# gildas-lormeau/zlib-streams-ts

Hardware: AMD Instinct MI355X
Metric: uncompressed MB/s, deflate-raw L6, 4096x64KiB batch at 1/2/4/8 GPUs (higher is better)
Workload: dtype u8; 1 GPU; 4096 x 65536 B text-corpus streams split across the GPUs, deflate-raw level 6; global_streams=4096, streams_per_gpu=4096, stream_bytes=65536, level=6, format=deflate-raw, compressed_bytes=91855591, parallelism=dp1

## Files before the change

zlib-streams-ts_amd/csrc/deflate_sweep.hip:

```cpp
#include <hip/hip_runtime.h>
#include "zs_common.h"
#include "zs_kernels.h"
#include "zs_sweep_ring.h"
#include "zs_sweep_long.h"
#include "zs_sweep_ends.h"
#include <type_traits>
#include <utility>

#define ZS_SW_WIN_WORDS ((ZS_SEG_WPOS + 258u + 20u + 3u) / 4u + 2u)
#define ZS_SW_RING 128u
#define ZS_SW_MW 320u
#ifndef ZS_SW_RUN_CAP
#define ZS_SW_RUN_CAP 16u
#endif

typedef __attribute__((address_space(3))) uint32_t zs_sw_lds_u32;
static __device__ __forceinline__ uint32_t sw_lds_addr(const void* p) {
  return (uint32_t)(uintptr_t)(const zs_sw_lds_u32*)p;
}

static __device__ __forceinline__ uint32_t sw_hash(uint32_t w) {
  return (((w & 0xffu) << 10) ^ (((w >> 8) & 0xffu) << 5) ^ ((w >> 16) & 0xffu)) & ZS_HASH_MASK;
}

#define ZS_BK_WPT (16384u / ZS_BK_THREADS)
#define ZS_BK_PPL (ZS_BK_THREADS / 64u)
#ifndef ZS_BK_PROF
#define ZS_BK_PROF 0
#endif
#if ZS_BK_PROF
__device__ unsigned long long zs_bk_stat[4];
extern "C" int zs_bucket_stats(unsigned long long* out) {
  return (int)hipMemcpyFromSymbol(out, HIP_SYMBOL(zs_bk_stat), sizeof(zs_bk_stat));
}
#define BK_MARK(i) do { if (threadIdx.x == 0) { const unsigned long long t_ = wall_clock64(); atomicAdd(&zs_bk_stat[i], t_ - bk_t); bk_t = t_; } } while (0)
#else
#define BK_MARK(i) do { } while (0)
#endif
#define ZS_BK_INFLIGHT 8
#define ZS_BK_CHUNK 2048u
#define ZS_BK_KEYS 256u
#define ZS_BK_HELPERS (ZS_BK_THREADS - 64u)
#define ZS_BK_EPT ((ZS_BK_CHUNK + ZS_BK_HELPERS - 1u) / ZS_BK_HELPERS)

static __device__ __forceinline__ void bk_lds_barrier() {
  asm volatile("s_waitcnt lgkmcnt(0)\n\ts_barrier" ::: "memory");
}

template <bool ORD>
__global__ __launch_bounds__(ZS_BK_THREADS) void zs_k_bucket(const uint8_t* __restrict__ in,
                                                            const uint64_t* __restrict__ in_off,
                                                            const uint32_t* __restrict__ in_len,
                                                            const uint64_t* __restrict__ pos_base,
                                                            const zs_sweep_seg* __restrict__ segs,
                                                            uint16_t* __restrict__ members, uint2* __restrict__ mres) {
  __shared__ uint32_t cnt[16384];
  __shared__ uint32_t part[ZS_BK_KEYS + ZS_BK_CHUNK / 2];
  static_assert(ZS_BK_KEYS + ZS_BK_CHUNK / 2 >= ZS_BK_THREADS, "part[] holds the scan's partial sums");
  __shared__ uint32_t stg[ZS_BK_CHUNK / 4 + 2];
  __shared__ uint16_t q[2][ZS_BK_CHUNK];
  const zs_sweep_seg G = segs[blockIdx.x];
  const int s = (int)G.s;
  const uint32_t nrel = in_len[s] - G.base;
  const uint32_t tid = threadIdx.x;
  const uint8_t* src = in + in_off[s] + G.base;
  uint16_t* mem = members + G.mb;
  uint2* out = mres + pos_base[s] + G.base;
  const uint32_t m = nrel > 2 ? min(nrel - 2, G.ohi) : 0u;
  const uint32_t n = min(nrel, m + 2u);
  if (nrel - m <= 2u)
    for (uint32_t p = m + tid; p < nrel; p += ZS_BK_THREADS) out[p] = make_uint2(0, 0);
  if (m == 0) return;
  for (uint32_t i = tid; i < 16384 / 4; i += ZS_BK_THREADS) reinterpret_cast<uint4*>(cnt)[i] = make_uint4(0, 0, 0, 0);
  const bool aligned = ((uintptr_t)src & 3u) == 0;
#if ZS_BK_PROF
  unsigned long long bk_t = wall_clock64();
  if (threadIdx.x == 0) atomicAdd(&zs_bk_stat[3], 1ull);
#endif
  __syncthreads();
  {
    uint32_t w[5], nw[5];
    auto load5 = [&](uint32_t p0, uint32_t* x) __attribute__((always_inline)) {
#pragma unroll
      for (int k = 0; k < 5; k++) x[k] = zs_load_word(src, n, p0 + 16 * tid + 4 * k);
    };
    load5(0, nw);
    for (uint32_t p0 = 0; p0 < m; p0 += 16 * ZS_BK_THREADS) {
#pragma unroll
      for (int k = 0; k < 5; k++) w[k] = nw[k];
      if (p0 + 16 * ZS_BK_THREADS < m) load5(p0 + 16 * ZS_BK_THREADS, nw);
#pragma unroll
      for (uint32_t j = 0; j < 16; j++) {
        const uint32_t p = p0 + 16 * tid + j;
        const uint32_t h = sw_hash(__builtin_amdgcn_alignbyte(w[(j >> 2) + 1], w[j >> 2], j & 3u));
        if (p < m) atomicAdd(&cnt[h >> 1], 1u << (16u * (h & 1u)));
      }
    }
  }
  __syncthreads();
  BK_MARK(0);
  {
    uint32_t sum = 0;
    for (uint32_t j = 0; j < ZS_BK_WPT; j++) {
      const uint32_t w = cnt[ZS_BK_WPT * tid + ((j + tid) & (ZS_BK_WPT - 1u))];
      sum += (w & 0xffffu) + (w >> 16);
    }
    part[tid] = sum;
    __syncthreads();
    if (tid < 64) {
      uint32_t v[ZS_BK_PPL], t = 0;
#pragma unroll
      for (uint32_t j = 0; j < ZS_BK_PPL; j++) { v[j] = part[ZS_BK_PPL * tid + j]; t += v[j]; }
      uint32_t x = t;
#pragma unroll
      for (int d = 1; d < 64; d <<= 1) {
        const uint32_t y = __shfl_up(x, d, 64);
        if (tid >= (uint32_t)d) x += y;
      }
      uint32_t run = x - t;
#pragma unroll
      for (uint32_t j = 0; j < ZS_BK_PPL; j++) { part[ZS_BK_PPL * tid + j] = run; run += v[j]; }
    }
    __syncthreads();
    uint32_t run = part[tid];
    for (uint32_t j = 0; j < ZS_BK_WPT; j++) {
      const uint32_t w = cnt[ZS_BK_WPT * tid + j];
      const uint32_t lo = w & 0xffffu;
      cnt[ZS_BK_WPT * tid + j] = run | ((run + lo) << 16);
      run += lo + (w >> 16);
    }
  }
  __syncthreads();
  BK_MARK(1);
  const uint32_t wave = tid >> 6, lane = tid & 63u;
  constexpr uint32_t PH = ZS_BK_CHUNK / (64 * ZS_BK_INFLIGHT);
  static_assert(PH == 4, "a chunk is four steps: count, scan, place, store");
  uint32_t* const kc = part;
  uint16_t* const srt = reinterpret_cast<uint16_t*>(part + ZS_BK_KEYS);
  if (tid < ZS_BK_KEYS) kc[tid] = 0;
  uint32_t sl[ZS_BK_EPT];
  const uint32_t ht = tid - 64u;
  constexpr uint32_t CW = ZS_BK_CHUNK / 4 / 64;
  uint32_t nxt[CW + 1];
  auto fetch = [&](uint32_t c0) {
#pragma unroll
    for (uint32_t i = 0; i <= CW; i++) {
      const uint32_t w = 64 * i + lane;
      const uint32_t at = c0 + 4 * w;
      uint32_t v = 0;
      if (w < ZS_BK_CHUNK / 4 + 2) {
        if (aligned && at + 4 <= n) v = *(const uint32_t*)(src + at);
        else
          for (uint32_t k = 0; k < 4; k++)
            if (at + k < n) v |= (uint32_t)src[at + k] << (8 * k);
      }
      nxt[i] = v;
    }
  };
  if (wave == 0) fetch(0);
  const uint32_t nch = (m + ZS_BK_CHUNK - 1) / ZS_BK_CHUNK;
  for (uint32_t c = 0; c <= nch; c++) {
    const uint32_t c0 = c * ZS_BK_CHUNK;
    const uint32_t c1 = min(m, c0 + ZS_BK_CHUNK);
    const uint32_t b0 = c0 - ZS_BK_CHUNK, cnt1 = min(m, c0) - b0;
    const uint16_t* const qp = q[(c - 1) & 1u];
#pragma unroll
    for (uint32_t ph = 0; ph < PH; ph++) {
    const uint32_t g0 = c0 + 64 * ZS_BK_INFLIGHT * ph;
    if (wave == 0 && c < nch) {
      if (ph == 0) {
        __builtin_amdgcn_s_waitcnt(0xc07f);
        __builtin_amdgcn_wave_barrier();
#pragma unroll
        for (uint32_t i = 0; i <= CW; i++)
          if (64 * i + lane < ZS_BK_CHUNK / 4 + 2) stg[64 * i + lane] = nxt[i];
        __builtin_amdgcn_s_waitcnt(0xc07f);
        __builtin_amdgcn_wave_barrier();
        if (c0 + ZS_BK_CHUNK < m) fetch(c0 + ZS_BK_CHUNK);
      }
      uint16_t* const qc = q[c & 1u];
      if (g0 < c1) {
        uint32_t a[ZS_BK_INFLIGHT], v[ZS_BK_INFLIGHT], sh[ZS_BK_INFLIGHT], e[ZS_BK_INFLIGHT], hh[ZS_BK_INFLIGHT];
#pragma unroll
        for (int j = 0; j < ZS_BK_INFLIGHT; j++) {
          const uint32_t p = g0 + 64 * j + lane;
          const uint32_t o = p - c0;
          const uint32_t h = sw_hash(__builtin_amdgcn_alignbyte(stg[(o >> 2) + 1], stg[o >> 2], o & 3u));
          hh[j] = h;
          sh[j] = 16u * (h & 1u);
          a[j] = sw_lds_addr(&cnt[h >> 1]);
          v[j] = p < c1 ? 1u << sh[j] : 0u;
        }
        if (!ORD) {
#pragma unroll
          for (int j = 0; j < ZS_BK_INFLIGHT; j++) {
            const uint32_t p = g0 + 64 * j + lane;
            const uint32_t h = hh[j];
            const uint64_t mm = zs_wave_match(h, p < c1);
            const uint32_t rank = (uint32_t)__builtin_popcountll(mm & ((1ull << lane) - 1ull));
            const uint32_t lead = mm ? (uint32_t)__builtin_ctzll(mm) : lane;
            uint32_t old = 0;
            if (p < c1 && lead == lane)
              old = atomicAdd(&cnt[h >> 1], (uint32_t)__builtin_popcountll(mm) << sh[j]);
            old = (uint32_t)__builtin_amdgcn_ds_bpermute((int)(lead * 4u), (int)old);
            e[j] = old + (rank << sh[j]);
          }
        } else {
        asm volatile(
            "ds_add_rtn_u32 %0, %8, %16\n\t"
            "ds_add_rtn_u32 %1, %9, %17\n\t"
            "ds_add_rtn_u32 %2, %10, %18\n\t"
            "ds_add_rtn_u32 %3, %11, %19\n\t"
            "ds_add_rtn_u32 %4, %12, %20\n\t"
            "ds_add_rtn_u32 %5, %13, %21\n\t"
            "ds_add_rtn_u32 %6, %14, %22\n\t"
            "ds_add_rtn_u32 %7, %15, %23\n\t"
            "s_waitcnt lgkmcnt(0)"
            : "=&v"(e[0]), "=&v"(e[1]), "=&v"(e[2]), "=&v"(e[3]), "=&v"(e[4]), "=&v"(e[5]), "=&v"(e[6]), "=&v"(e[7])
            : "v"(a[0]), "v"(a[1]), "v"(a[2]), "v"(a[3]), "v"(a[4]), "v"(a[5]), "v"(a[6]), "v"(a[7]), "v"(v[0]),
              "v"(v[1]), "v"(v[2]), "v"(v[3]), "v"(v[4]), "v"(v[5]), "v"(v[6]), "v"(v[7])
            : "memory");
        }
#pragma unroll
        for (int j = 0; j < ZS_BK_INFLIGHT; j++) {
          const uint32_t p = g0 + 64 * j + lane;
          if (p < c1) qc[p - c0] = (uint16_t)(e[j] >> sh[j]);
        }
      }
    } else if (wave != 0 && c > 0) {
      if (ph == 0) {
#pragma unroll
        for (uint32_t k = 0; k < ZS_BK_EPT; k++) {
          const uint32_t o = ht + ZS_BK_HELPERS * k;
          sl[k] = o < cnt1 ? (uint32_t)qp[o] : 0u;
          if (o < cnt1) atomicAdd(&kc[sl[k] >> 8], 1u);
        }
      } else if (ph == 1) {
        if (wave == 1) {
          constexpr uint32_t KPL = ZS_BK_KEYS / 64u;
          uint32_t v[KPL], t = 0;
#pragma unroll
          for (uint32_t j = 0; j < KPL; j++) { v[j] = kc[KPL * lane + j]; t += v[j]; }
          uint32_t x = t;
#pragma unroll
          for (int d = 1; d < 64; d <<= 1) {
            const uint32_t y = __shfl_up(x, d, 64);
            if (lane >= (uint32_t)d) x += y;
          }
          uint32_t run = x - t;
#pragma unroll
          for (uint32_t j = 0; j < KPL; j++) { kc[KPL * lane + j] = run; run += v[j]; }
        }
      } else if (ph == 2) {
#pragma unroll
        for (uint32_t k = 0; k < ZS_BK_EPT; k++) {
          const uint32_t o = ht + ZS_BK_HELPERS * k;
          if (o < cnt1) srt[atomicAdd(&kc[sl[k] >> 8], 1u)] = (uint16_t)o;
        }
      } else {
        for (uint32_t i = ht; i < cnt1; i += ZS_BK_HELPERS) {
          const uint32_t o = srt[i];
          mem[qp[o]] = (uint16_t)(b0 + o);
        }
        if (ht < ZS_BK_KEYS) kc[ht] = 0;
      }
    }
    bk_lds_barrier();
    }
  }
  BK_MARK(2);
}
template __global__ void zs_k_bucket<true>(const uint8_t*, const uint64_t*, const uint32_t*, const uint64_t*,
                                           const zs_sweep_seg*, uint16_t*, uint2*);
template __global__ void zs_k_bucket<false>(const uint8_t*, const uint64_t*, const uint32_t*, const uint64_t*,
                                            const zs_sweep_seg*, uint16_t*, uint2*);

static __device__ __forceinline__ uint32_t sw_word(const uint32_t* win, uint32_t off) {
  const uint32_t i = off >> 2;
  return __builtin_amdgcn_alignbyte(win[i + 1], win[i], off & 3u);
}

static __device__ __forceinline__ uint32_t sw_extend(const uint32_t* win, uint32_t p, uint32_t q, uint32_t maxc,
                                                     uint32_t from) {
  uint32_t k = from;
  while (k < maxc) {
    const uint32_t y = sw_word(win, q + k) ^ sw_word(win, p + k);
    if (y) { k += (uint32_t)(__builtin_ctz(y) >> 3); break; }
    k += 4;
  }
  return k < maxc ? k : maxc;
}

static __device__ __forceinline__ uint32_t max3(uint32_t a, uint32_t b, uint32_t c) {
  return max(max(a, b), c);
}

static __device__ __forceinline__ uint32_t sw_x7(uint32_t w) {
  const uint32_t b0 = w & 0xffu, b1 = (w >> 8) & 0xffu;
  return ((b0 >> 5) & 3u) | ((b1 & 7u) << 2) | (((b1 >> 5) & 3u) << 5);
}
template <bool A7>
struct SwSig;
template <>
struct SwSig<false> {
  static constexpr uint32_t LONG = 88u;
  static constexpr uint32_t THR0 = 23u;
  static constexpr uint32_t EXT = 11u;
  uint32_t a, b, c;
  static __device__ __forceinline__ uint4 rec(const uint32_t* win, uint32_t q, uint32_t w0) {
    return make_uint4(w0, sw_word(win, q + 4), sw_word(win, q + 8) & 0x00ffffffu, 0u);
  }
  __device__ __forceinline__ uint32_t mbits(uint32_t x, uint32_t y, uint32_t z) const {
    uint32_t f0, f1, f2;
    asm("v_ffbl_b32 %0, %1" : "=v"(f0) : "v"(x ^ a));
    asm("v_ffbl_b32 %0, %1\n\tv_add_u32_e64 %0, %0, 32 clamp" : "=&v"(f1) : "v"(y ^ b));
    asm("v_ffbl_b32 %0, %1\n\tv_add_u32_e32 %0, 64, %0" : "=&v"(f2) : "v"(z ^ c));
    return min(min(f0, f1), f2);
  }
  template <uint32_t U>
  __device__ __forceinline__ uint32_t step(uint32_t x, uint32_t y, uint32_t z) const {
    return (mbits(x, y, z) & ~7u) | (7u - U);
  }
  template <uint32_t U>
  __device__ __forceinline__ uint32_t step(uint32_t x, uint32_t y, uint32_t z, uint64_t lm) const {
    uint32_t r;
    asm("v_cndmask_b32_e64 %0, 0, %1, %2" : "=v"(r) : "v"(step<U>(x, y, z)), "s"(lm));
    return r;
  }
  static __device__ __forceinline__ uint32_t len(uint32_t sigma) { return sigma; }
};
template <>
struct SwSig<true> {
  static constexpr uint32_t LONG = 64u;
  static constexpr uint32_t THR0 = 7u;
  static constexpr uint32_t EXT = 10u;
  uint32_t a, b;
  static __device__ __forceinline__ uint4 rec(const uint32_t* win, uint32_t q, uint32_t w0) {
    return make_uint4(sw_x7(w0) | (sw_word(win, q + 3) << 8), sw_word(win, q + 6), sw_word(win, q + EXT), 0u);
  }
  __device__ __forceinline__ uint32_t mbits(uint32_t x, uint32_t y, uint32_t) const {
    uint32_t f0, f1;
    asm("v_ffbl_b32 %0, %1" : "=v"(f0) : "v"(x ^ a));
    asm("v_ffbl_b32 %0, %1\n\tv_add_u32_e64 %0, %0, 32 clamp" : "=&v"(f1) : "v"(y ^ b));
    return min(min(f0, f1), 64u);
  }
  template <uint32_t U>
  __device__ __forceinline__ uint32_t step(uint32_t x, uint32_t y, uint32_t) const {
    uint32_t t;
    asm("v_xor_b32_e32 %0, %0, %3\n\t"
        "v_xor_b32_e32 %1, %2, %4\n\t"
        "v_ffbl_b32 %0, %0\n\t"
        "v_ffbl_b32 %1, %1\n\t"
        "v_add_u32_e64 %1, %1, 32 clamp\n\t"
        "v_min3_u32 %0, %0, %1, 64\n\t"
        "v_and_or_b32 %0, %0, -8, %5"
        : "+v"(x), "=v"(t)
        : "v"(y), "v"(a), "v"(b), "n"(7u - U));
    return x;
  }
  template <uint32_t U>
  __device__ __forceinline__ uint32_t step(uint32_t x, uint32_t y, uint32_t, uint64_t lm) const {
    uint32_t t;
    asm("v_xor_b32_e32 %0, %0, %3\n\t"
        "v_xor_b32_e32 %1, %2, %4\n\t"
        "v_ffbl_b32 %0, %0\n\t"
        "v_ffbl_b32 %1, %1\n\t"
        "v_add_u32_e64 %1, %1, 32 clamp\n\t"
        "v_min3_u32 %0, %0, %1, 64\n\t"
        "v_and_or_b32 %0, %0, -8, %5\n\t"
        "v_cndmask_b32_e64 %0, 0, %0, %6"
        : "+v"(x), "=v"(t)
        : "v"(y), "v"(a), "v"(b), "n"(7u - U), "s"(lm));
    return x;
  }
  static __device__ __forceinline__ uint32_t len(uint32_t sigma) { return sigma ? sigma + 2u : 2u; }
};

struct SwRing {
  uint2 ab[2 * ZS_SW_RING];
  uint32_t c[2 * ZS_SW_RING];
  uint32_t key[2 * ZS_SW_RING];
  __device__ __forceinline__ void put(int b, uint32_t lane, uint4 r) {
    const uint32_t i = (uint32_t)(64 * b + (int)lane) & (ZS_SW_RING - 1);
    ab[i] = make_uint2(r.x, r.y);
    ab[i + ZS_SW_RING] = make_uint2(r.x, r.y);
    c[i] = r.z;
    c[i + ZS_SW_RING] = r.z;
    key[i] = r.w;
    key[i + ZS_SW_RING] = r.w;
  }
  static __device__ __forceinline__ uint32_t base(int c, uint32_t s, uint32_t lane) {
    return ((uint32_t)(64 * (c - (int)s - 1) + (int)lane) & (ZS_SW_RING - 1)) + 64u * s + 64u;
  }
};
struct SwRingP {
  uint2 ab[ZS_SWR_SLOTS + ZS_SWR_MIRROR];
  uint32_t c[ZS_SWR_SLOTS + ZS_SWR_MIRROR];
  uint32_t key[ZS_SWR_SLOTS + ZS_SWR_MIRROR];
  __device__ __forceinline__ void put(int b, uint32_t lane, uint4 r) {
    const uint32_t i = zs_swr_block_slot(b) + lane;
    ab[i] = make_uint2(r.x, r.y);
    c[i] = r.z;
    key[i] = r.w;
    if (zs_swr_mirrored(b)) {
      ab[i + ZS_SWR_SLOTS] = make_uint2(r.x, r.y);
      c[i + ZS_SWR_SLOTS] = r.z;
      key[i + ZS_SWR_SLOTS] = r.w;
    }
  }
  static __device__ __forceinline__ uint32_t base(int c, uint32_t s, uint32_t lane) { return zs_swr_base(c, s) + lane; }
  __device__ __forceinline__ uint32_t pos(int c, uint32_t lane, uint32_t t) const {
    return key[zs_swr_member_slot(c, lane, t)] & 0xffffu;
  }
};

#ifndef ZS_SW_PROF
#define ZS_SW_PROF 0
#endif
#if ZS_SW_PROF
__device__ unsigned long long zs_sw_stat[8];
#define SW_STAT(i, v) do { if ((threadIdx.x & 63u) == __builtin_ctzll(__builtin_amdgcn_read_exec())) atomicAdd(&zs_sw_stat[i], (unsigned long long)(v)); } while (0)
extern "C" int zs_sw_stats(unsigned long long* out) {
  return (int)hipMemcpyFromSymbol(out, HIP_SYMBOL(zs_sw_stat), sizeof(zs_sw_stat));
}
#else
#define SW_STAT(i, v) do { } while (0)
#endif

template <class F, uint32_t... U>
static __device__ __forceinline__ void sw_each_(F&& f, std::integer_sequence<uint32_t, U...>) {
  (f(std::integral_constant<uint32_t, U>{}), ...);
}
template <uint32_t N, class F>
static __device__ __forceinline__ void sw_each(F&& f) {
  sw_each_(f, std::make_integer_sequence<uint32_t, N>{});
}
template <uint32_t N>
static __device__ __forceinline__ uint32_t sw_gmax(const uint32_t* sc) {
  static_assert(N == 8 || N == 4 || N == 3 || N == 1, "group sizes");
  if constexpr (N == 8) return max(max3(sc[0], sc[1], sc[2]), max3(sc[3], sc[4], max3(sc[5], sc[6], sc[7])));
  else if constexpr (N == 4) return max3(sc[0], sc[1], max(sc[2], sc[3]));
  else if constexpr (N == 3) return max3(sc[0], sc[1], sc[2]);
  else return sc[0];
}

template <bool A7>
struct SwLane {
  SwSig<A7> S;
  uint32_t p;
  bool own;
  uint32_t maxc, nice;
  uint32_t khead, klim;
  uint32_t long_m;
  uint32_t own_ext;
  uint32_t thr, bt, thr_s, bt_s;
  uint32_t lthr, lbt, lthr_s, lbt_s;
  uint64_t alive_m;
  uint32_t head;
  bool snapped;
  __device__ __forceinline__ bool tail() const { return maxc <= 12u; }
  __device__ __forceinline__ void snap() {
    thr_s = thr;
    bt_s = bt;
    lthr_s = lthr;
    lbt_s = lbt;
    snapped = true;
  }
};

template <bool A7, bool MW, bool PR, bool U8>
struct SwWave {
  using Sig = SwSig<A7>;
  using Lane = SwLane<A7>;
  using Ring = std::conditional_t<PR, SwRingP, SwRing>;
  const uint32_t* win;
  Ring* R;
  uint16_t* mw;
  const uint16_t* mem;
  uint32_t n, m, lane;
  uint32_t budget, budget_s, nice_cfg;
  int cc;
  zs_swr_range vr;
  int mw0;

  __device__ __forceinline__ int k() const { return 64 * cc + (int)lane; }
  __device__ __forceinline__ uint32_t fetch(int j) const { return j >= 0 && (uint32_t)j < m ? (uint32_t)mem[j] : 0u; }
  __device__ __forceinline__ uint4 make_rec(uint32_t q) const {
    const uint32_t w0 = sw_word(win, q);
    uint4 r = Sig::rec(win, q, w0);
    r.w = (sw_hash(w0) << 16) | q;
    return r;
  }
  __device__ __forceinline__ void build_blk(int blk, uint32_t q) {
    const int j = 64 * blk + (int)lane;
    const bool in = j >= 0 && (uint32_t)j < m;
    if (MW && (uint32_t)(j - mw0) < ZS_SW_MW) mw[j - mw0] = (uint16_t)q;
    R->put(blk, lane, in ? make_rec(q) : make_uint4(0, 0, 0, 0));
    if constexpr (PR) vr = zs_swr_extend(vr, blk);
  }
  __device__ __forceinline__ bool missing(int blk) const { return !PR || !zs_swr_has(vr, blk); }
  __device__ __forceinline__ uint32_t member(uint32_t t) const {
    if constexpr (PR) return R->pos(cc, lane, t);
    const int j = k() - (int)t;
    return MW ? (uint32_t)mw[j - mw0] : (uint32_t)mem[j];
  }

  __device__ __forceinline__ uint4 start(Lane& L, uint32_t p, bool mem_ok, bool own) const {
    const uint4 rown = mem_ok ? make_rec(p) : make_uint4(0, 0, 0, 0);
    L.S.a = rown.x;
    L.S.b = rown.y;
    if constexpr (!A7) L.S.c = rown.z | 0x01000000u;
    L.own_ext = A7 ? rown.z : sw_word(win, p + Sig::EXT);
    L.p = p;
    L.own = own;
    const uint32_t h = rown.w >> 16;
    const uint32_t look = n - p;
    L.maxc = look < ZS_MAX_MATCH ? look : ZS_MAX_MATCH;
    L.nice = look < nice_cfg ? look : nice_cfg;
    L.long_m = L.tail() ? 0xffffu : Sig::LONG;
    const uint32_t limit = p > ZS_MAX_DIST ? p - ZS_MAX_DIST : 0u;
    L.khead = (h << 16) | (limit > 1u ? limit : 1u);
    L.klim = (h << 16) | limit;
    L.thr = L.thr_s = Sig::THR0;
    L.bt = L.bt_s = 0;
    L.lthr = L.lthr_s = ZS_SWL_NONE;
    L.lbt = L.lbt_s = 0;
    L.alive_m = 0;
    L.head = 0;
    L.snapped = budget_s <= 1u;
    return rown;
  }

  __device__ __forceinline__ void build(uint4 rown, uint32_t p, uint32_t qb, bool have_qb) {
    mw0 = 64 * cc - (int)budget;
    if (MW) mw[k() - mw0] = (uint16_t)p;
    __builtin_amdgcn_s_waitcnt(0xc07f);
    __builtin_amdgcn_wave_barrier();
    R->put(cc, lane, rown);
    if constexpr (PR) vr = zs_swr_push(vr, cc);
    if (missing(cc - 1)) build_blk(cc - 1, have_qb ? qb : fetch(k() - 64));
    __builtin_amdgcn_s_waitcnt(0xc07f);
    __builtin_amdgcn_wave_barrier();
  }

  __device__ __forceinline__ void fold(Lane& L, uint32_t gm, uint32_t t0, const uint32_t* sc, uint32_t cnt,
                                       const uint32_t* gc, const uint32_t* gk) const {
    const bool up = gm > (L.thr | 7u);
    L.thr = up ? gm : L.thr;
    L.bt = up ? t0 : L.bt;
    if (__builtin_expect(__builtin_amdgcn_ballot_w64(gm >= L.long_m) != 0, 0)) {
      SW_STAT(3, 1);
      auto lscore = [&](uint32_t u) -> uint32_t {
        const uint32_t ls = cnt - 1u - u;
        const uint32_t x = (A7 ? gc[ls] : sw_word(win, (gk[ls] & 0xffffu) + Sig::EXT)) ^ L.own_ext;
        const uint32_t len = x ? Sig::EXT + ((uint32_t)__builtin_ctz(x) >> 3)
                               : sw_extend(win, L.p, gk[ls] & 0xffffu, L.maxc, Sig::EXT + 4u);
        return zs_swl_score(len, L.maxc, L.nice, u);
      };
      const bool lg = gm >= L.long_m && zs_swl_open(L.lthr, L.nice);
      uint32_t w[2] = {0, 0};
#pragma unroll
      for (uint32_t u = 0; u < 8; u++)
        if (u < cnt) w[u >> 2] |= sc[u] << (8u * (u & 3u));
      constexpr uint32_t LB = (0x80u - Sig::LONG) * 0x01010101u;
      const uint32_t nl = (uint32_t)__builtin_popcount((w[0] + LB) & 0x80808080u) +
                          (uint32_t)__builtin_popcount((w[1] + LB) & 0x80808080u);
      const uint64_t twice = __builtin_amdgcn_ballot_w64(lg && nl > 1u);
      uint32_t gl = 0;
      const uint32_t u1 = zs_swl_first(gm);
      if (lg) gl = lscore(u1);
      if (__builtin_expect(twice != 0, 0)) {
        if ((twice >> lane) & 1u) {
          uint32_t lm = 0;
#pragma unroll
          for (uint32_t u = 0; u < 8; u++) lm |= (u < cnt && sc[u] >= L.long_m) ? 1u << u : 0u;
          lm &= ~(1u << u1);
          while (lm) {
            gl = zs_swl_join(gl, lscore((uint32_t)__builtin_ctz(lm)));
            lm &= lm - 1u;
          }
        }
      }
      zs_swl_fold(gl, t0, &L.lthr, &L.lbt);
    }
  }

  struct Grp {
    const uint2* A;
    const uint32_t *C, *K;
  };
  template <uint32_t N>
  __device__ __forceinline__ Grp at(uint32_t base, uint32_t t0) const {
    const uint32_t lo = base - (t0 + (N - 1u));
    return Grp{R->ab + lo, R->c + lo, R->key + lo};
  }
  __device__ __forceinline__ const uint32_t* c_of(const Grp& g) const {
    if constexpr (A7) return R->c + ((sw_lds_addr(g.A) - sw_lds_addr(R->ab)) >> 3);
    else return g.C;
  }
  template <uint32_t N>
  __device__ __forceinline__ void group_fast(Lane& L, const Grp& g, uint32_t t0) const {
    uint32_t sc[N];
    sw_each<N>([&](auto uc) __attribute__((always_inline)) {
      constexpr uint32_t u = decltype(uc)::value;
      const uint2 ab = g.A[N - 1u - u];
      sc[u] = L.S.template step<u>(ab.x, ab.y, A7 ? 0u : g.C[N - 1u - u]);
    });
    const uint32_t gm = __builtin_amdgcn_inverse_ballot_w64(L.alive_m) ? sw_gmax<N>(sc) : 0u;
    fold(L, gm, t0, sc, N, c_of(g), g.K);
  }
  template <uint32_t N, bool HEAD>
  __device__ __forceinline__ void group_masked(Lane& L, const Grp& g, uint32_t t0) const {
    uint32_t sc[N], key[N];
    uint2 ab[N];
#pragma unroll
    for (uint32_t u = 0; u < N; u++) {
      key[u] = g.K[N - 1u - u];
      ab[u] = g.A[N - 1u - u];
    }
    if constexpr (HEAD) {
      const bool a1 = L.own && key[0] >= L.khead;
      L.head = a1 ? 1u | ((L.p - (key[0] & 0xffffu)) == ZS_MAX_DIST ? 0x8000u : 0u) : 0u;
      L.alive_m = __builtin_amdgcn_ballot_w64(a1);
    }
    uint64_t lm = L.alive_m;
    sw_each<N>([&](auto uc) __attribute__((always_inline)) {
      constexpr uint32_t u = decltype(uc)::value;
      if (!HEAD || u) {
        uint64_t gt;
        const uint32_t ku = key[u], klim = L.klim;
        asm("v_cmp_gt_u32_e64 %0, %1, %2" : "=s"(gt) : "v"(ku), "v"(klim));
        lm = gt & L.alive_m;
      }
      sc[u] = L.S.template step<u>(ab[u].x, ab[u].y, A7 ? 0u : g.C[N - 1u - u], lm);
    });
    L.alive_m = lm;
    fold(L, sw_gmax<N>(sc), t0, sc, N, c_of(g), g.K);
  }

  template <bool HEAD>
  __device__ __forceinline__ uint64_t ends(const Lane& L, const uint32_t* K, uint64_t a0, uint64_t last,
                                           uint32_t gm) const {
    const uint64_t part = a0 & ~last;
    const uint64_t raise = __builtin_amdgcn_ballot_w64(zs_swe_raises(gm, L.thr)) & part;
    uint64_t bad = __builtin_amdgcn_ballot_w64(zs_swe_long(gm, L.long_m)) & part;
    if (raise) {
      SW_STAT(5, 1);
      const uint32_t wk = ((const zs_sw_lds_u32*)K)[zs_swe_winner_slot(gm)];
      bad |= raise & ~__builtin_amdgcn_ballot_w64(zs_swe_winner_live(gm, wk, L.klim, HEAD));
    }
    return bad;
  }
  template <bool HEAD>
  __device__ __forceinline__ uint32_t remask(const Lane& L, const uint32_t* K, uint64_t a0, uint32_t* sc) const {
    SW_STAT(HEAD ? 7 : 6, 1);
    uint32_t key[8];
#pragma unroll
    for (uint32_t u = HEAD ? 1u : 0u; u < 8; u++) key[u] = K[7u - u];
    sw_each<8>([&](auto uc) __attribute__((always_inline)) {
      constexpr uint32_t u = decltype(uc)::value;
      if (!HEAD || u) {
        uint64_t gt;
        const uint32_t ku = key[u], klim = L.klim;
        asm("v_cmp_gt_u32_e64 %0, %1, %2" : "=s"(gt) : "v"(ku), "v"(klim));
        uint32_t v;
        const uint32_t su = sc[u];
        asm("v_cndmask_b32_e64 %0, 0, %1, %2" : "=v"(v) : "v"(su), "s"(gt));
        sc[u] = v;
      }
    });
    return __builtin_amdgcn_inverse_ballot_w64(a0) ? sw_gmax<8>(sc) : 0u;
  }

  __device__ __forceinline__ void open8(Lane& L, const Grp& g) const {
    const uint32_t k1 = g.K[7], k8 = g.K[0];
    uint32_t sc[8];
    sw_each<8>([&](auto uc) __attribute__((always_inline)) {
      constexpr uint32_t u = decltype(uc)::value;
      const uint2 ab = g.A[7u - u];
      sc[u] = L.S.template step<u>(ab.x, ab.y, A7 ? 0u : g.C[7u - u]);
    });
    const bool a1 = L.own && k1 >= L.khead;
    L.head = a1 ? 1u | ((L.p - (k1 & 0xffffu)) == ZS_MAX_DIST ? 0x8000u : 0u) : 0u;
    const uint64_t a0 = __builtin_amdgcn_ballot_w64(a1);
    const uint64_t last = __builtin_amdgcn_ballot_w64(k8 > L.klim) & a0;
    uint32_t gm = a1 ? sw_gmax<8>(sc) : 0u;
    uint64_t bad = 0;
    if (last != a0) bad = ends<true>(L, g.K, a0, last, gm);
    if (__builtin_expect(bad != 0, 0)) gm = remask<true>(L, g.K, a0, sc);
    L.alive_m = last;
    fold(L, gm, 1u, sc, 8u, c_of(g), g.K);
  }

  __device__ __forceinline__ void run(Lane& L, uint32_t base, uint32_t ta, uint32_t tb) const {
    auto last_of = [&](uint32_t t0) __attribute__((always_inline)) {
      uint32_t t1 = t0 + 7u <= tb ? t0 + 7u : t0 + 3u;
      if (t0 <= budget_s && t1 > budget_s) t1 = budget_s;
      return t1;
    };
    if (ta > tb) return;
    uint32_t t0 = ta, t1 = last_of(ta);
    uint32_t kl = R->key[base - t1];
    while (L.alive_m) {
      const uint64_t last_live = __builtin_amdgcn_ballot_w64(kl > L.klim) & L.alive_m;
      const uint32_t n0 = t1 + 1u, n1 = n0 <= tb ? last_of(n0) : t1;
      kl = R->key[base - n1];
      SW_STAT(last_live == L.alive_m ? 1 : 2, 1);
      SW_STAT(4, t1 - t0 + 1u);
      if (last_live == L.alive_m) {
        if (t1 - t0 == 7u) group_fast<8>(L, at<8>(base, t0), t0);
        else group_fast<4>(L, at<4>(base, t0), t0);
      } else {
        if (t1 - t0 == 7u) group_masked<8, false>(L, at<8>(base, t0), t0);
        else group_masked<4, false>(L, at<4>(base, t0), t0);
      }
      if (t1 == budget_s) L.snap();
      if (n0 > tb) break;
      t0 = n0;
      t1 = n1;
    }
  }

  __device__ __forceinline__ void run8(Lane& L, uint32_t base, uint32_t ta, uint32_t te) const {
    asm("" : "+s"(L.alive_m));
    Grp g = at<8>(base, ta);
    const zs_sw_lds_u32* k8 = (const zs_sw_lds_u32*)(g.K - 8);
    uint32_t kl = g.K[0];
    if (!L.alive_m) return;
    uint32_t t0 = ta;
    do {
      const uint64_t last_live = __builtin_amdgcn_ballot_w64(kl > L.klim) & L.alive_m;
      kl = k8[0];
      g.K = (const uint32_t*)(k8 + 8);
      SW_STAT(last_live == L.alive_m ? 1 : 2, 1);
      SW_STAT(4, 8u);
      const uint64_t a0 = L.alive_m;
      uint32_t sc[8];
      sw_each<8>([&](auto uc) __attribute__((always_inline)) {
        constexpr uint32_t u = decltype(uc)::value;
        const uint2 ab = g.A[7u - u];
        sc[u] = L.S.template step<u>(ab.x, ab.y, A7 ? 0u : g.C[7u - u]);
        if (u & 1u) __builtin_amdgcn_sched_barrier(0x180);
      });
      uint32_t gm = __builtin_amdgcn_inverse_ballot_w64(a0) ? sw_gmax<8>(sc) : 0u;
      uint64_t bad = 0;
      if (last_live != a0) {
        bad = ends<false>(L, g.K, a0, last_live, gm);
        L.alive_m = last_live;
      }
      asm("" : "+s"(bad));
      if (__builtin_expect(bad != 0, 0)) gm = remask<false>(L, g.K, a0, sc);
      fold(L, gm, t0, sc, 8u, c_of(g), g.K);
      t0 += 8u;
      g.A -= 8;
      if (!A7) g.C -= 8;
      k8 -= 8;
      asm("" : "+v"(k8));
    } while (t0 <= te && L.alive_m);
  }

  __device__ __forceinline__ void sweep(Lane& L) {
    const uint32_t base0 = Ring::base(cc, 0u, lane);
    const bool open8 = U8 || (budget_s >= 8u && budget >= 8u);
    if (open8) {
      if constexpr (U8) this->open8(L, at<8>(base0, 1u));
      else group_masked<8, true>(L, at<8>(base0, 1u), 1u);
      if (budget_s == 8u) L.snap();
    } else if constexpr (!U8) {
      group_masked<1, true>(L, at<1>(base0, 1u), 1u);
      if (budget_s == 1u) L.snap();
      if (budget >= 4u) {
        group_masked<3, false>(L, at<3>(base0, 2u), 2u);
        if (budget_s == 4u) L.snap();
      }
    }
    for (uint32_t b = 0; budget > 4u && L.alive_m; b++) {
      const int blk = cc - (int)b - 1;
      if (b >= 1 && missing(blk)) {
        __builtin_amdgcn_s_waitcnt(0xc07f);
        __builtin_amdgcn_wave_barrier();
        build_blk(blk, fetch(64 * blk + (int)lane));
        __builtin_amdgcn_s_waitcnt(0xc07f);
        __builtin_amdgcn_wave_barrier();
      }
      uint32_t ta = b == 0 ? (open8 ? 9u : 5u) : 64u * b + 1u;
      const uint32_t tb = min(64u * b + 64u, budget);
      const uint32_t base = Ring::base(cc, b, lane);
      if constexpr (U8) {
        while (ta <= tb && L.alive_m) {
          const bool cut = !L.snapped && budget_s <= tb;
          const uint32_t te = cut ? budget_s : tb;
          run8(L, base, ta, te);
          if (cut) L.snap();
          ta = te + 1u;
        }
      } else {
        run(L, base, ta, tb);
      }
      if (tb >= budget) break;
    }
    if (!L.snapped) L.snap();
  }

  __device__ __forceinline__ void settle(const Lane& L, uint2* out) const {
    __builtin_amdgcn_s_waitcnt(0xc07f);
    __builtin_amdgcn_wave_barrier();
    if (!L.own) return;
    const uint32_t p = L.p;
    uint32_t rx = 0, ry = 0;
    if (L.head) {
      uint32_t len = 2, dist = 0, len_s = 2, dist_s = 0;
      if (L.tail()) {
        const int k = this->k();
        uint32_t b = 2u << 16, bs = 2u << 16;
        for (uint32_t t = 1; t <= budget && (int)t <= k; t++) {
          const uint32_t q = member(t);
          const uint32_t key = (sw_hash(sw_word(win, q)) << 16) | q;
          if (t == 1u ? key < L.khead : key <= L.klim) break;
          uint32_t len = 12;
          for (uint32_t o = 0; o < 12u; o += 4) {
            const uint32_t y = sw_word(win, q + o) ^ sw_word(win, p + o);
            if (y) { len = o + (uint32_t)(__builtin_ctz(y) >> 3); break; }
          }
          const uint32_t sc = ((len < L.maxc ? len : L.maxc) << 16) | (0xffffu - t);
          b = max(b, sc);
          if (t <= budget_s) bs = max(bs, sc);
        }
        len = b >> 16;
        dist = len > 2u ? p - (uint32_t)mem[k - (int)(0xffffu - (b & 0xffffu))] : 0u;
        len_s = bs >> 16;
        dist_s = len_s > 2u ? p - (uint32_t)mem[k - (int)(0xffffu - (bs & 0xffffu))] : 0u;
      } else {
        const uint32_t tb = L.bt + 7u - (L.thr & 7u), tb_s = L.bt_s + 7u - (L.thr_s & 7u);
        if (L.bt) {
          len = Sig::len(L.thr >> 3);
          dist = p - member(tb);
        }
        if (L.bt_s) {
          len_s = Sig::len(L.thr_s >> 3);
          dist_s = tb_s == tb ? dist : p - member(tb_s);
        }
        auto long_of = [&](uint32_t lt, uint32_t t, uint32_t& ln, uint32_t& ds) {
          const uint32_t q = member(t);
          ln = lt >> 3;
          if (ln >= L.nice) ln = sw_extend(win, p, q, L.maxc, Sig::EXT);
          ds = p - q;
        };
        if (L.lbt) long_of(L.lthr, L.lbt, len, dist);
        if (L.lbt_s) {
          if (L.lbt_s == L.lbt) {
            len_s = len;
            dist_s = dist;
          } else {
            long_of(L.lthr_s, L.lbt_s, len_s, dist_s);
          }
        }
      }
      rx = (len << 16) | (len > 2u ? dist : 0u) | (L.head & 0x8000u);
      ry = (len_s << 16) | (len_s > 2u ? dist_s : 0u);
    }
    out[p] = make_uint2(rx, ry);
  }
};

template <bool A7, bool MW, bool PR, bool U8>
static __device__ __forceinline__ void sw_body(const uint32_t* win, void* ringp, uint16_t* mw, uint32_t* next,
                                               uint32_t n, uint32_t m, uint32_t olo, uint32_t ohi,
                                               const uint16_t* mem, uint2* out, int chain, int nice_cfg) {
  using Wave = SwWave<A7, MW, PR, U8>;
  const uint32_t lane = threadIdx.x & 63u;
  Wave W{win, (typename Wave::Ring*)ringp, mw, mem, n, m, lane, (uint32_t)chain, (uint32_t)chain >> 2,
         (uint32_t)nice_cfg, 0, zs_swr_empty(), 0};
  const uint32_t nchunks = (m + 63) / 64;
  auto claim = [&]() -> uint32_t {
    uint32_t c = 0;
    if (lane == 0) c = atomicAdd(next, 1u);
    return __builtin_amdgcn_readfirstlane(c);
  };
  auto claim_run = [&](uint32_t& c0, uint32_t& c1) {
    uint32_t a = 0, r = 0;
    if (lane == 0) {
      const uint32_t cur = __hip_atomic_load(next, __ATOMIC_RELAXED, __HIP_MEMORY_SCOPE_WORKGROUP);
      r = zs_swr_run_len(cur < nchunks ? nchunks - cur : 0u, ZS_SW_RUN_CAP);
      a = atomicAdd(next, r);
    }
    c0 = __builtin_amdgcn_readfirstlane(a);
    c1 = min(c0 + (uint32_t)__builtin_amdgcn_readfirstlane(r), nchunks);
  };
  uint32_t c, ce = 0;
  if constexpr (PR) claim_run(c, ce);
  else c = claim();
  uint32_t pf_p = W.fetch((int)(64 * c + lane)), pf_b = W.fetch((int)(64 * c + lane) - 64);
  bool fresh_n = true;
  for (;;) {
    if (c >= nchunks) break;
    const bool fresh = fresh_n;
    uint32_t cn, cen = ce;
    if constexpr (PR) {
      cn = c + 1u;
      fresh_n = cn >= ce;
      if (fresh_n) claim_run(cn, cen);
      if (fresh) W.vr = zs_swr_empty();
    } else {
      cn = claim();
    }
    W.cc = (int)c;
    const bool mem_ok = (uint32_t)W.k() < m;
    SW_STAT(0, 1);
    const uint32_t p = pf_p, qb = pf_b;
    if (cn < nchunks) {
      pf_p = W.fetch((int)(64 * cn + lane));
      if (!PR || fresh_n) pf_b = W.fetch((int)(64 * cn + lane) - 64);
    }
    c = cn;
    ce = cen;
    const bool own = mem_ok && p >= olo && p < ohi;
    if (__builtin_amdgcn_ballot_w64(own) == 0) {
      W.vr = zs_swr_empty();
      continue;
    }
    typename Wave::Lane L;
    const uint4 rown = W.start(L, p, mem_ok, own);
    W.build(rown, p, qb, fresh);
    W.sweep(L);
    W.settle(L, out);
  }
}

template <bool U8>
__global__ __launch_bounds__(1024) void zs_k_sweep(const uint8_t* __restrict__ in, const uint64_t* __restrict__ in_off,
                                                   const uint32_t* __restrict__ in_len,
                                                   const uint64_t* __restrict__ pos_base,
                                                   const zs_sweep_seg* __restrict__ segs,
                                                   const uint16_t* __restrict__ members, uint2* __restrict__ mres,
                                                   int chain, int nice_cfg) {
  constexpr uint32_t RING_BYTES = 16u * sizeof(SwRing), MWIN_BYTES = 16u * ZS_SW_MW * sizeof(uint16_t);
  static_assert(16u * sizeof(SwRingP) <= RING_BYTES + MWIN_BYTES, "the persistent rings must fit the old ones' LDS");
  __shared__ __attribute__((aligned(16))) uint8_t rmem[RING_BYTES + MWIN_BYTES];
  __shared__ __attribute__((aligned(16))) uint32_t win[ZS_SW_WIN_WORDS];
  __shared__ uint32_t next;
  const zs_sweep_seg G = segs[blockIdx.x];
  const int s = (int)G.s;
  const uint32_t n = in_len[s] - G.base;
  if (n < 3) return;
  const uint32_t m = min(n - 2, G.ohi);
  const uint8_t* src = in + in_off[s] + G.base;
  uint32_t hi = 0;
  if ((((uintptr_t)src) & 15u) == 0) {
    for (uint32_t i = threadIdx.x; 4 * i < ZS_SW_WIN_WORDS; i += 1024) {
      const uint32_t b = 16 * i;
      uint4 v;
      if (b + 16 <= n) v = ((const uint4*)src)[i];
      else {
        uint32_t t[4] = {0, 0, 0, 0};
        for (uint32_t k = 0; k < 16; k++)
          if (b + k < n) t[k >> 2] |= (uint32_t)src[b + k] << (8 * (k & 3));
        v = make_uint4(t[0], t[1], t[2], t[3]);
      }
      hi |= v.x | v.y | v.z | v.w;
      if (4 * i + 3 < ZS_SW_WIN_WORDS) *(uint4*)(win + 4 * i) = v;
      else for (uint32_t k = 0; 4 * i + k < ZS_SW_WIN_WORDS; k++) win[4 * i + k] = (&v.x)[k];
    }
  } else {
    for (uint32_t i = threadIdx.x; i < ZS_SW_WIN_WORDS; i += 1024) {
      uint32_t v = 0;
      for (uint32_t k = 0; k < 4; k++)
        if (4 * i + k < n) v |= (uint32_t)src[4 * i + k] << (8 * k);
      hi |= v;
      win[i] = v;
    }
  }
  if (threadIdx.x == 0) next = 0;
  const bool a7 = !__syncthreads_or((hi & 0x80808080u) != 0);
  const uint32_t wave = threadIdx.x >> 6;
  const uint16_t* mem = members + G.mb;
  uint2* out = mres + pos_base[s] + G.base;
  const uint32_t olo = G.olo, ohi = G.ohi;
  if (chain <= (int)ZS_SWR_MAX_CHAIN) {
    SwRingP* const R = reinterpret_cast<SwRingP*>(rmem) + wave;
    if (a7) sw_body<true, false, true, U8>(win, R, nullptr, &next, n, m, olo, ohi, mem, out, chain, nice_cfg);
    else sw_body<false, false, true, U8>(win, R, nullptr, &next, n, m, olo, ohi, mem, out, chain, nice_cfg);
    return;
  }
  SwRing* const R = reinterpret_cast<SwRing*>(rmem) + wave;
  uint16_t* const mw = reinterpret_cast<uint16_t*>(rmem + RING_BYTES) + wave * ZS_SW_MW;
  if (chain + 64 <= (int)ZS_SW_MW) {
    if (a7) sw_body<true, true, false, U8>(win, R, mw, &next, n, m, olo, ohi, mem, out, chain, nice_cfg);
    else sw_body<false, true, false, U8>(win, R, mw, &next, n, m, olo, ohi, mem, out, chain, nice_cfg);
  } else {
    if (a7) sw_body<true, false, false, U8>(win, R, mw, &next, n, m, olo, ohi, mem, out, chain, nice_cfg);
    else sw_body<false, false, false, U8>(win, R, mw, &next, n, m, olo, ohi, mem, out, chain, nice_cfg);
  }
}
template __global__ void zs_k_sweep<true>(const uint8_t*, const uint64_t*, const uint32_t*, const uint64_t*,
                                          const zs_sweep_seg*, const uint16_t*, uint2*, int, int);
template __global__ void zs_k_sweep<false>(const uint8_t*, const uint64_t*, const uint32_t*, const uint64_t*,
                                           const zs_sweep_seg*, const uint16_t*, uint2*, int, int);
```

Before: 23290 MB/s.

## Move bucket hashing to helper waves and store slots in lane-major 16-byte layout

The hash computation and input staging move off wave 0 onto the last helper threads. Those threads prefetch input words into registers, compute hashes one step ahead, and publish them through a small double-buffered LDS queue. Wave 0 then only reads one 16-byte vector of precomputed hash keys, runs the atomic claims, and writes its eight slots as a single 16-byte store in a permuted layout that the sorting helpers decode with a bit permutation. This shortens wave 0's critical path and widens its LDS accesses, at the cost of extra register state in the hasher threads and a more intricate cross-wave schedule.

```diff
diff --git a/zlib-streams-ts_amd/csrc/deflate_sweep.hip b/zlib-streams-ts_amd/csrc/deflate_sweep.hip
--- a/zlib-streams-ts_amd/csrc/deflate_sweep.hip
+++ b/zlib-streams-ts_amd/csrc/deflate_sweep.hip
@@ -57,8 +57,8 @@
   __shared__ uint32_t cnt[16384];
   __shared__ uint32_t part[ZS_BK_KEYS + ZS_BK_CHUNK / 2];
   static_assert(ZS_BK_KEYS + ZS_BK_CHUNK / 2 >= ZS_BK_THREADS, "part[] holds the scan's partial sums");
-  __shared__ uint32_t stg[ZS_BK_CHUNK / 4 + 2];
-  __shared__ uint16_t q[2][ZS_BK_CHUNK];
+  __shared__ __attribute__((aligned(16))) uint16_t hq[2][64 * ZS_BK_INFLIGHT];
+  __shared__ __attribute__((aligned(16))) uint16_t q[2][ZS_BK_CHUNK];
   const zs_sweep_seg G = segs[blockIdx.x];
   const int s = (int)G.s;
   const uint32_t nrel = in_len[s] - G.base;
@@ -72,7 +72,6 @@
     for (uint32_t p = m + tid; p < nrel; p += ZS_BK_THREADS) out[p] = make_uint2(0, 0);
   if (m == 0) return;
   for (uint32_t i = tid; i < 16384 / 4; i += ZS_BK_THREADS) reinterpret_cast<uint4*>(cnt)[i] = make_uint4(0, 0, 0, 0);
-  const bool aligned = ((uintptr_t)src & 3u) == 0;
 #if ZS_BK_PROF
   unsigned long long bk_t = wall_clock64();
   if (threadIdx.x == 0) atomicAdd(&zs_bk_stat[3], 1ull);
@@ -130,34 +129,57 @@
       run += lo + (w >> 16);
     }
   }
+  const uint32_t wave = tid >> 6, lane = tid & 63u;
+  constexpr uint32_t STEP = 64 * ZS_BK_INFLIGHT;
+  constexpr uint32_t PH = ZS_BK_CHUNK / STEP;
+  static_assert(PH == 4, "a chunk is four steps: count, scan, place, store");
+  static_assert(ZS_BK_INFLIGHT == 8, "a lane's hash words and slots of a step are one 16-byte access");
+  static_assert(ZS_BK_HELPERS >= 64 + STEP / 2, "the hashing waves: two positions per thread, wave 1 scans");
+  uint32_t* const kc = part;
+  uint16_t* const srt = reinterpret_cast<uint16_t*>(part + ZS_BK_KEYS);
+  uint32_t sl[ZS_BK_EPT];
+  const uint32_t ht = tid - 64u;
+  auto bk_qpos = [](uint32_t e) { return (e & ~(STEP - 1u)) | ((e & 7u) << 6) | ((e >> 3) & 63u); };
+  const bool hasher = tid >= ZS_BK_THREADS - STEP / 2;
+  const uint32_t hi = tid - (ZS_BK_THREADS - STEP / 2);
+  const uint32_t hj = (hi >> 2) & 7u, hl = 8u * (hi >> 5) + 2u * (hi & 3u);
+  uint32_t hw[PH][2] = {}, nw[PH][2] = {};
+  const bool aligned = ((uintptr_t)src & 3u) == 0;
+  auto hload = [&](uint32_t c0) __attribute__((always_inline)) {
+    const uint32_t at = c0 + ((64u * hj + hl) & ~3u);
+    if (aligned && c0 + ZS_BK_CHUNK + 4 <= n) {
+#pragma unroll
+      for (uint32_t i = 0; i < PH; i++)
+#pragma unroll
+        for (uint32_t k = 0; k < 2; k++) nw[i][k] = *reinterpret_cast<const uint32_t*>(src + at + STEP * i + 4 * k);
+    } else {
+#pragma unroll
+      for (uint32_t i = 0; i < PH; i++)
+#pragma unroll
+        for (uint32_t k = 0; k < 2; k++) nw[i][k] = zs_load_word(src, n, at + STEP * i + 4 * k);
+    }
+  };
+  auto hwait = [&]() __attribute__((always_inline)) {
+    asm volatile("" : "+v"(nw[0][0]), "+v"(nw[0][1]), "+v"(nw[1][0]), "+v"(nw[1][1]), "+v"(nw[2][0]), "+v"(nw[2][1]),
+                 "+v"(nw[3][0]), "+v"(nw[3][1]));
+#pragma unroll
+    for (uint32_t i = 0; i < PH; i++) { hw[i][0] = nw[i][0]; hw[i][1] = nw[i][1]; }
+  };
+  auto hput = [&](const uint32_t* w, uint32_t buf) __attribute__((always_inline)) {
+#pragma unroll
+    for (uint32_t k = 0; k < 2; k++) {
+      const uint32_t h = sw_hash(__builtin_amdgcn_alignbyte(w[1], w[0], (hl & 2u) + k));
+      hq[buf][ZS_BK_INFLIGHT * (hl + k) + hj] = (uint16_t)(((h >> 1) << 2) | (h & 1u));
+    }
+  };
+  if (hasher) {
+    hload(0);
+    hwait();
+    hput(hw[0], 0);
+  }
   __syncthreads();
   BK_MARK(1);
-  const uint32_t wave = tid >> 6, lane = tid & 63u;
-  constexpr uint32_t PH = ZS_BK_CHUNK / (64 * ZS_BK_INFLIGHT);
-  static_assert(PH == 4, "a chunk is four steps: count, scan, place, store");
-  uint32_t* const kc = part;
-  uint16_t* const srt = reinterpret_cast<uint16_t*>(part + ZS_BK_KEYS);
   if (tid < ZS_BK_KEYS) kc[tid] = 0;
-  uint32_t sl[ZS_BK_EPT];
-  const uint32_t ht = tid - 64u;
-  constexpr uint32_t CW = ZS_BK_CHUNK / 4 / 64;
-  uint32_t nxt[CW + 1];
-  auto fetch = [&](uint32_t c0) {
-#pragma unroll
-    for (uint32_t i = 0; i <= CW; i++) {
-      const uint32_t w = 64 * i + lane;
-      const uint32_t at = c0 + 4 * w;
-      uint32_t v = 0;
-      if (w < ZS_BK_CHUNK / 4 + 2) {
-        if (aligned && at + 4 <= n) v = *(const uint32_t*)(src + at);
-        else
-          for (uint32_t k = 0; k < 4; k++)
-            if (at + k < n) v |= (uint32_t)src[at + k] << (8 * k);
-      }
-      nxt[i] = v;
-    }
-  };
-  if (wave == 0) fetch(0);
   const uint32_t nch = (m + ZS_BK_CHUNK - 1) / ZS_BK_CHUNK;
   for (uint32_t c = 0; c <= nch; c++) {
     const uint32_t c0 = c * ZS_BK_CHUNK;
@@ -166,74 +188,73 @@
     const uint16_t* const qp = q[(c - 1) & 1u];
 #pragma unroll
     for (uint32_t ph = 0; ph < PH; ph++) {
-    const uint32_t g0 = c0 + 64 * ZS_BK_INFLIGHT * ph;
-    if (wave == 0 && c < nch) {
-      if (ph == 0) {
-        __builtin_amdgcn_s_waitcnt(0xc07f);
-        __builtin_amdgcn_wave_barrier();
-#pragma unroll
-        for (uint32_t i = 0; i <= CW; i++)
-          if (64 * i + lane < ZS_BK_CHUNK / 4 + 2) stg[64 * i + lane] = nxt[i];
-        __builtin_amdgcn_s_waitcnt(0xc07f);
-        __builtin_amdgcn_wave_barrier();
-        if (c0 + ZS_BK_CHUNK < m) fetch(c0 + ZS_BK_CHUNK);
-      }
-      uint16_t* const qc = q[c & 1u];
-      if (g0 < c1) {
-        uint32_t a[ZS_BK_INFLIGHT], v[ZS_BK_INFLIGHT], sh[ZS_BK_INFLIGHT], e[ZS_BK_INFLIGHT], hh[ZS_BK_INFLIGHT];
+    const uint32_t g0 = c0 + STEP * ph;
+    if (ph == PH - 1) hwait();
+    if (wave == 0) {
+      auto claim = [&](auto full, const uint4 hv) __attribute__((always_inline)) {
+        constexpr bool FULL = decltype(full)::value;
+        const uint32_t hx[ZS_BK_INFLIGHT / 2] = {hv.x, hv.y, hv.z, hv.w};
+        uint32_t a[ZS_BK_INFLIGHT], v[ZS_BK_INFLIGHT], sh[ZS_BK_INFLIGHT], e[ZS_BK_INFLIGHT], xx[ZS_BK_INFLIGHT];
 #pragma unroll
         for (int j = 0; j < ZS_BK_INFLIGHT; j++) {
-          const uint32_t p = g0 + 64 * j + lane;
-          const uint32_t o = p - c0;
-          const uint32_t h = sw_hash(__builtin_amdgcn_alignbyte(stg[(o >> 2) + 1], stg[o >> 2], o & 3u));
-          hh[j] = h;
-          sh[j] = 16u * (h & 1u);
-          a[j] = sw_lds_addr(&cnt[h >> 1]);
-          v[j] = p < c1 ? 1u << sh[j] : 0u;
+          const uint32_t x = (j & 1) ? hx[j >> 1] >> 16 : hx[j >> 1] & 0xffffu;
+          xx[j] = x;
+          sh[j] = 16u * (x & 1u);
+          a[j] = sw_lds_addr(cnt) + (x & 0xfffcu);
+          v[j] = FULL || g0 + 64 * j + lane < c1 ? 1u << sh[j] : 0u;
         }
         if (!ORD) {
 #pragma unroll
           for (int j = 0; j < ZS_BK_INFLIGHT; j++) {
-            const uint32_t p = g0 + 64 * j + lane;
-            const uint32_t h = hh[j];
-            const uint64_t mm = zs_wave_match(h, p < c1);
+            const bool in = FULL || g0 + 64 * j + lane < c1;
+            const uint64_t mm = zs_wave_match(xx[j], in);
             const uint32_t rank = (uint32_t)__builtin_popcountll(mm & ((1ull << lane) - 1ull));
             const uint32_t lead = mm ? (uint32_t)__builtin_ctzll(mm) : lane;
             uint32_t old = 0;
-            if (p < c1 && lead == lane)
-              old = atomicAdd(&cnt[h >> 1], (uint32_t)__builtin_popcountll(mm) << sh[j]);
+            if (in && lead == lane) old = atomicAdd(&cnt[xx[j] >> 2], (uint32_t)__builtin_popcountll(mm) << sh[j]);
             old = (uint32_t)__builtin_amdgcn_ds_bpermute((int)(lead * 4u), (int)old);
             e[j] = old + (rank << sh[j]);
           }
         } else {
-        asm volatile(
-            "ds_add_rtn_u32 %0, %8, %16\n\t"
-            "ds_add_rtn_u32 %1, %9, %17\n\t"
-            "ds_add_rtn_u32 %2, %10, %18\n\t"
-            "ds_add_rtn_u32 %3, %11, %19\n\t"
-            "ds_add_rtn_u32 %4, %12, %20\n\t"
-            "ds_add_rtn_u32 %5, %13, %21\n\t"
-            "ds_add_rtn_u32 %6, %14, %22\n\t"
-            "ds_add_rtn_u32 %7, %15, %23\n\t"
-            "s_waitcnt lgkmcnt(0)"
-            : "=&v"(e[0]), "=&v"(e[1]), "=&v"(e[2]), "=&v"(e[3]), "=&v"(e[4]), "=&v"(e[5]), "=&v"(e[6]), "=&v"(e[7])
-            : "v"(a[0]), "v"(a[1]), "v"(a[2]), "v"(a[3]), "v"(a[4]), "v"(a[5]), "v"(a[6]), "v"(a[7]), "v"(v[0]),
-              "v"(v[1]), "v"(v[2]), "v"(v[3]), "v"(v[4]), "v"(v[5]), "v"(v[6]), "v"(v[7])
-            : "memory");
-        }
-#pragma unroll
-        for (int j = 0; j < ZS_BK_INFLIGHT; j++) {
-          const uint32_t p = g0 + 64 * j + lane;
-          if (p < c1) qc[p - c0] = (uint16_t)(e[j] >> sh[j]);
-        }
-      }
-    } else if (wave != 0 && c > 0) {
+          asm volatile(
+              "ds_add_rtn_u32 %0, %8, %16\n\t"
+              "ds_add_rtn_u32 %1, %9, %17\n\t"
+              "ds_add_rtn_u32 %2, %10, %18\n\t"
+              "ds_add_rtn_u32 %3, %11, %19\n\t"
+              "ds_add_rtn_u32 %4, %12, %20\n\t"
+              "ds_add_rtn_u32 %5, %13, %21\n\t"
+              "ds_add_rtn_u32 %6, %14, %22\n\t"
+              "ds_add_rtn_u32 %7, %15, %23\n\t"
+              "s_waitcnt lgkmcnt(0)"
+              : "=&v"(e[0]), "=&v"(e[1]), "=&v"(e[2]), "=&v"(e[3]), "=&v"(e[4]), "=&v"(e[5]), "=&v"(e[6]), "=&v"(e[7])
+              : "v"(a[0]), "v"(a[1]), "v"(a[2]), "v"(a[3]), "v"(a[4]), "v"(a[5]), "v"(a[6]), "v"(a[7]), "v"(v[0]),
+                "v"(v[1]), "v"(v[2]), "v"(v[3]), "v"(v[4]), "v"(v[5]), "v"(v[6]), "v"(v[7])
+              : "memory");
+        }
+        uint32_t sw[ZS_BK_INFLIGHT / 2];
+#pragma unroll
+        for (int k = 0; k < ZS_BK_INFLIGHT / 2; k++)
+          sw[k] = ((e[2 * k] >> sh[2 * k]) & 0xffffu) | ((e[2 * k + 1] >> sh[2 * k + 1]) << 16);
+        *reinterpret_cast<uint4*>(&q[c & 1u][STEP * ph + ZS_BK_INFLIGHT * lane]) = make_uint4(sw[0], sw[1], sw[2], sw[3]);
+      };
+      if (g0 < c1) {
+        const uint4 hv = *reinterpret_cast<const uint4*>(&hq[ph & 1u][ZS_BK_INFLIGHT * lane]);
+        if (c1 - g0 >= STEP) claim(std::true_type{}, hv);
+        else claim(std::false_type{}, hv);
+      }
+    } else {
+      if (hasher && c < nch) {
+        hput(hw[(ph + 1u) % PH], (ph + 1u) & 1u);
+        if (ph == 0 && c + 1 < nch) hload(c0 + ZS_BK_CHUNK);
+      }
+      if (c > 0) {
       if (ph == 0) {
 #pragma unroll
         for (uint32_t k = 0; k < ZS_BK_EPT; k++) {
-          const uint32_t o = ht + ZS_BK_HELPERS * k;
-          sl[k] = o < cnt1 ? (uint32_t)qp[o] : 0u;
-          if (o < cnt1) atomicAdd(&kc[sl[k] >> 8], 1u);
+          const uint32_t e = ht + ZS_BK_HELPERS * k;
+          const bool in = bk_qpos(e) < cnt1;
+          sl[k] = in ? (uint32_t)qp[e] : 0u;
+          if (in) atomicAdd(&kc[sl[k] >> 8], 1u);
         }
       } else if (ph == 1) {
         if (wave == 1) {
@@ -254,15 +275,16 @@
       } else if (ph == 2) {
 #pragma unroll
         for (uint32_t k = 0; k < ZS_BK_EPT; k++) {
-          const uint32_t o = ht + ZS_BK_HELPERS * k;
-          if (o < cnt1) srt[atomicAdd(&kc[sl[k] >> 8], 1u)] = (uint16_t)o;
+          const uint32_t e = ht + ZS_BK_HELPERS * k;
+          if (bk_qpos(e) < cnt1) srt[atomicAdd(&kc[sl[k] >> 8], 1u)] = (uint16_t)e;
         }
       } else {
         for (uint32_t i = ht; i < cnt1; i += ZS_BK_HELPERS) {
-          const uint32_t o = srt[i];
-          mem[qp[o]] = (uint16_t)(b0 + o);
+          const uint32_t e = srt[i];
+          mem[qp[e]] = (uint16_t)(b0 + bk_qpos(e));
         }
         if (ht < ZS_BK_KEYS) kc[ht] = 0;
+      }
       }
     }
     bk_lds_barrier();
```

Result: no change. 23430 MB/s (median of 6 runs) (+0.6%).
